# aynik/carta1

Hardware: AMD Instinct MI355X
Metric: atrac1_stereo_frames_per_s_encode (higher is better)
Workload: dtype f32+f64

## Files before the change

### carta1_amd/csrc/c1_api.hip

```cpp
#include <algorithm>
#include <cmath>
#include <cstdarg>
#include <cstdio>
#include <cstdlib>
#include <cstring>
#include <limits>
#include <map>
#include <memory>
#include <atomic>
#include <mutex>
#include <string>
#include <thread>
#include <vector>

#include "c1_internal.h"
#include "c1_detect_bound.h"

#pragma clang fp contract(off)

namespace {

#include "c1_default_tables.inc"

thread_local std::string g_error;
// ... 617 lines not shown
  const bool all_long_modes = !detect && opts->fixed_block_modes[0] == 0 && opts->fixed_block_modes[1] == 0 &&
                              opts->fixed_block_modes[2] == 0 && !getenv("C1_NO_FAST_LONG");
  const bool all_short_modes = !detect && opts->fixed_block_modes[0] != 0 && opts->fixed_block_modes[1] != 0 &&
                               opts->fixed_block_modes[2] != 0;
  bool speculate = (all_long_modes || all_short_modes) && !taps && units && ctx->spec_tables_ok && ctx->spec_mode != 0;
  bool quantize32 = !taps && units && ctx->spec_tables_ok && ctx->spec_mode != 0;
  static const bool det_spec_env_off = getenv("C1_DETECT_SPEC") && atoi(getenv("C1_DETECT_SPEC")) == 0;
  bool detect_spec = detect && !taps && ctx->spec_tables_ok && ctx->spec_mode != 0 && !det_spec_env_off;
  if (ctx->spec_mode == 1 && frames * channels < kSpecMinUnits) speculate = quantize32 = detect_spec = false;
  const bool overlap = speculate && ctx->overlap && ctx->s_tail != nullptr;
  if (!overlap && (rc = join_tail(ctx))) return rc;
  const bool piped = ctx->pipeline && !taps && frames > chunk && !speculate;
  hipStream_t sA = piped ? ctx->s_ana : ctx->stream, sB = piped ? ctx->s_rest : ctx->stream;
  if (piped) {
    HIP_TRY(hipEventRecord(ctx->ev_in, ctx->stream));
    HIP_TRY(hipStreamWaitEvent(sA, ctx->ev_in, 0));
    HIP_TRY(hipStreamWaitEvent(sB, ctx->ev_in, 0));
  }
  int64_t index = 0;
  for (int64_t f0 = 0, n = 0; f0 < frames; f0 += n, ++index) {
    n = taps ? frames : std::min(chunk, frames - f0);
    int p = piped ? (int)(index & 1) : 0;
    if (overlap) { p = ctx->ws_next; ctx->ws_next ^= 1; }
    C1EncodeLaunch L;
    memset(&L, 0, sizeof L);
    for (int c = 0; c < channels; c++) L.pcm[c] = pcm[c] + f0 * 512;
    L.channels = channels;
    L.frames = n;
    L.halo_frames = (int)std::min<int64_t>(2, f0 + halo_frames);
    L.tables = ctx->d_tables;
    L.opts = ctx->d_opts;
    L.coefs = taps ? coefs_tap : ctx->d_coefs[p];
    L.side = taps ? side_tap : ctx->d_side[p];
    L.alloc = taps ? alloc_tap : ctx->d_alloc[p];
    L.cand = ctx->d_cand[p];
    L.work_count = ctx->d_work[p];
    L.work_list = ctx->d_work[p] + 4;
    L.sel_list = ctx->d_work[p] + 4 + (size_t)ctx->ws_units * 7;
    L.bands = bands ? bands + f0 * channels * 512 : nullptr;
    L.units = units ? units + f0 * channels * C1_UNIT_BYTES : nullptr;
    const bool all_long = all_long_modes;
    if (piped && index >= 2) HIP_TRY(hipStreamWaitEvent(sA, ctx->ev_free[p], 0));
    if (speculate) {
      L.eps = ctx->d_eps[p];
      bind_lists(ctx, p, &L);
      if (ctx->spec_mode == 1) { bind_defer(ctx, p, &L); L.spec_defer = ctx->spec_defer; }
      if (c1k_pick_run(n, channels, 0) <= 64 && !getenv("C1_NO_SF_PREPASS"))
        L.open_masks = reinterpret_cast<unsigned long long *>((reinterpret_cast<uintptr_t>(ctx->d_redo[p] + kListHead + 3 * (size_t)ctx->ws_units + (size_t)ctx->ws_units / 4 + 4) + 7) & ~(uintptr_t)7);
      if (overlap && ctx->tail_used[p]) HIP_TRY(hipStreamWaitEvent(sA, ctx->ev_tail[p], 0));
      HIP_TRY(hipMemsetAsync(ctx->d_redo[p], 0, kListHead * sizeof(uint32_t), sA));
      {
        ScopedTiming t(ctx, K_ANALYSIS, sA);
        c1k_launch_analysis_spec(L, all_short_modes, sA);
        if (L.defer_list) {
          C1EncodeLaunch D = L;
          uint32_t *dense = ctx->d_redo[p] + kListHead + 2 * (size_t)ctx->ws_units;
          c1k_launch_defer_compact(L, dense, ctx->d_redo[p] + 3, sA);
          D.unit_list = dense;
          D.unit_count = ctx->d_redo[p] + 3;
          D.list_runs = 1;
          D.defer_list = nullptr;
          if (all_long_modes) c1k_launch_analysis_long(D, sA); else c1k_launch_analysis(D, false, sA);
        }
      }
      if (L.open_masks) {
        ScopedTiming t(ctx, K_REDO, sA);
        {
          C1EncodeLaunch X = L;
          uint32_t *open_list = ctx->d_redo[p] + kListHead + 2 * (size_t)ctx->ws_units;
          c1k_launch_open_compact(L, open_list, ctx->d_redo[p] + 5, sA);
          X.unit_list = open_list;
          X.unit_count = ctx->d_redo[p] + 5;
          X.list_runs = 0;
          X.list_zero_eps = 1;
          X.defer_list = nullptr;
          X.open_masks = nullptr;
          if (all_long_modes) c1k_launch_analysis_long(X, sA); else c1k_launch_analysis(X, false, sA);
        }
      }
      { ScopedTiming t(ctx, K_ALLOCATE, sA); c1k_launch_allocate(L, sA); }
      if (overlap && ctx->tail_used[p ^ 1]) HIP_TRY(hipStreamWaitEvent(sA, ctx->ev_tail[p ^ 1], 0));
      { ScopedTiming t(ctx, K_PACK, sA); c1k_launch_pack_spec(L, all_long_modes, sA); }
      hipStream_t sT = sA;
      if (overlap) {
        sT = ctx->s_tail;
        HIP_TRY(hipEventRecord(ctx->ev_main[p], sA));
        HIP_TRY(hipStreamWaitEvent(sT, ctx->ev_main[p], 0));
      }
      {
        ScopedTiming t(ctx, K_REDO, sT);
        hipStream_t sA = sT;
        C1EncodeLaunch R = L;
        R.defer_list = nullptr;
        R.unit_list = L.reana_list;
        R.unit_count = L.reana_count;
        if (all_long_modes) c1k_launch_analysis_long(R, sA); else c1k_launch_analysis(R, false, sA);
        if (!L.open_masks) {
          C1EncodeLaunch A = R;
          A.unit_list = L.realloc_list;
          A.unit_count = L.realloc_count;
          c1k_launch_allocate(A, sA);
        }
        R.unit_list = L.redo_list;
        R.unit_count = L.redo_count;
        c1k_launch_pack(R, all_long_modes, sA);
        c1k_launch_spec_totals(ctx->d_spec_totals, (uint64_t)(n * channels), ctx->d_redo[p], 0, sA);
      }
      if (overlap) {
        HIP_TRY(hipEventRecord(ctx->ev_tail[p], sT));
        ctx->tail_used[p] = true;
        ctx->tail_pending = true;
      }
      continue;
    }
    {
      ScopedTiming t(ctx, K_ANALYSIS, sA);
      if (all_long) c1k_launch_analysis_long(L, sA);
      else if (detect) {
        c1k_launch_detect(L, ctx->d_bands[p], ctx->d_feat[p], ctx->d_modes[p], ctx->d_lists[p], detect_spec, nullptr, sA);
        if (detect_spec) c1k_launch_spec_totals(ctx->d_spec_totals, (uint64_t)(n * channels), ctx->d_lists[p] + 2, 2, sA);
        if (L.bands) HIP_TRY(hipMemcpyAsync(L.bands, ctx->d_bands[p] + (size_t)channels * 512, (size_t)n * channels * 512 * sizeof(float),
                                            hipMemcpyDeviceToDevice, sA));
      } else c1k_launch_analysis(L, false, sA);
    }
// ... 2787 lines not shown
```

### carta1_amd/csrc/c1_device.h

```cpp
#pragma once
#include "c1_internal.h"

#include <algorithm>
#include <type_traits>

#pragma clang fp contract(off)

#define C1_WAVE 64

typedef const __attribute__((address_space(4))) C1DevTables *TablesPtr;
#define C1_TABLES(p) ((TablesPtr)(p))
__device__ __forceinline__ int lane_for_this_frame(int lane) {
  asm volatile("" : "+v"(lane));
  return lane;
}
__device__ __forceinline__ void wave_fence() {
  __builtin_amdgcn_fence(__ATOMIC_ACQ_REL, "wavefront");
  __builtin_amdgcn_wave_barrier();
}

__device__ __forceinline__ bool own_block() {
  int one = 1;
  asm volatile("" : "+s"(one));
  return one != 0;
// ... 10 lines not shown
__constant__ const uint8_t kSpecs[52] = {8, 8, 8, 8, 4,  4,  4,  4,  8,  8,  8,  8,  6,  6,  6,  6,  6,  6,
                                   6, 6, 6, 6, 6,  6,  7,  7,  7,  7,  9,  9,  9,  9,  10, 10, 10, 10,
                                   12, 12, 12, 12, 12, 12, 12, 12, 20, 20, 20, 20, 20, 20, 20, 20};
__constant__ const uint16_t kStartLong[52] = {0,   8,   16,  24,  32,  36,  40,  44,  48,  56,  64,  72,  80,
                                        86,  92,  98,  104, 110, 116, 122, 128, 134, 140, 146, 152, 159,
                                        166, 173, 180, 189, 198, 207, 216, 226, 236, 246, 256, 268, 280,
                                        292, 304, 316, 328, 340, 352, 372, 392, 412, 432, 452, 472, 492};
__constant__ const uint16_t kStartShort[52] = {0,   32,  64,  96,  8,   40,  72,  104, 12,  44,  76,  108, 20,
                                         52,  84,  116, 26,  58,  90,  122, 128, 160, 192, 224, 134, 166,
                                         198, 230, 141, 173, 205, 237, 150, 182, 214, 246, 256, 288, 320,
                                         352, 384, 416, 448, 480, 268, 300, 332, 364, 396, 428, 460, 492};
__constant__ const uint16_t kBfuFirst[53] = {0,   8,   16,  24,  32,  36,  40,  44,  48,  56,  64,  72,  80,  86,
                                       92,  98,  104, 110, 116, 122, 128, 134, 140, 146, 152, 159, 166, 173,
                                       180, 189, 198, 207, 216, 226, 236, 246, 256, 268, 280, 292, 304, 316,
                                       328, 340, 352, 372, 392, 412, 432, 452, 472, 492, 512};
__device__ __forceinline__ int bfu_amount(int index) { return index == 0 ? 20 : 24 + 4 * index; }

__device__ __forceinline__ int wl_bits(int wl) { return wl == 0 ? 0 : wl + 1; }
__device__ __forceinline__ int band_of_bfu(int b) { return b >= 36 ? 2 : (b >= 20 ? 1 : 0); }
__device__ __forceinline__ int bfu_of_slot(int p) {
  if (p < 32) return p >> 3;
  if (p < 48) return 4 + ((p - 32) >> 2);
  if (p < 80) return 8 + ((p - 48) >> 3);
  if (p < 152) return 12 + (p - 80) / 6;
  if (p < 180) return 24 + (p - 152) / 7;
  if (p < 216) return 28 + (p - 180) / 9;
  if (p < 256) return 32 + (p - 216) / 10;
  if (p < 352) return 36 + (p - 256) / 12;
  return 44 + (p - 352) / 20;
}

__device__ __forceinline__ float f32(double x) { return (float)x; }
typedef float v4f __attribute__((ext_vector_type(4)));

__device__ __forceinline__ int32_t to_int32(double x) {
  const double t = trunc(x);
  if (fabs(t) < 2147483648.0) return (int32_t)t;
  const uint64_t bits = (uint64_t)__double_as_longlong(t);
  const int e = (int)((bits >> 52) & 0x7ff);
  if (e == 0x7ff) return 0;
  const int sh = e - 1075;
  const uint64_t mant = (bits & 0xfffffffffffffull) | (1ull << 52);
  uint32_t low;
  if (sh >= 32) low = 0u;
  else if (sh >= 0) low = (uint32_t)(mant << sh);
  else low = (uint32_t)(mant >> (-sh));
  return (int32_t)((bits >> 63) ? (0u - low) : low);
}


template <int S = 5>
__device__ __forceinline__ int pidx(int e) { return e + ((e >> S) << 1); }

template <int D, int S>
__device__ __forceinline__ const double2 *qmf_window(const double *w, int lane, int u) {
  if constexpr (2 * D == (1 << S)) return reinterpret_cast<const double2 *>(w + (2 * D + 2) * lane + (2 * u + 2 * ((2 * u) >> S)));
  else return reinterpret_cast<const double2 *>(&w[pidx<S>(2 * D * lane + 2 * u)]);
}
template <int D, int S = 5>
__device__ __forceinline__ void qmf_analysis_core(const double *w, int lane, TablesPtr T,
                                                  double (&even)[D], double (&odd)[D]) {
#pragma unroll
  for (int d = 0; d < D; d++) even[d] = odd[d] = 0.0;
#pragma unroll
  for (int u = 22 + D; u >= 0; --u) {
    const double2 x = *qmf_window<D, S>(w, lane, u);
#pragma unroll
    for (int d = 0; d < D; d++) {
      const int j = d + 23 - u;
      if (j >= 0 && j < 24) {
        odd[d] = __builtin_fma(x.x, T->tap_e[23 - j], odd[d]);
        even[d] = __builtin_fma(x.y, T->tap_e[j], even[d]);
      }
    }
  }
}
template <int D, int S = 5>
__device__ __forceinline__ void qmf_synthesis_core(const double *w, int lane, TablesPtr T,
                                                   double (&s0)[D], double (&s1)[D]) {
#pragma unroll
  for (int d = 0; d < D; d++) s0[d] = s1[d] = 0.0;
#pragma unroll
  for (int u = 0; u <= 22 + D; ++u) {
    const double2 x = *qmf_window<D, S>(w, lane, u);
#pragma unroll
    for (int d = 0; d < D; d++) {
      const int j = u - d;
      if (j >= 0 && j < 24) {
        s0[d] = __builtin_fma(x.x, T->tap_e[j], s0[d]);
        s1[d] = __builtin_fma(x.y, T->tap_e[23 - j], s1[d]);
      }
    }
  }
}

__device__ __forceinline__ int wave_inclusive_scan(int x) {
  x += __builtin_amdgcn_update_dpp(0, x, 0x111, 0xf, 0xf, false);
  x += __builtin_amdgcn_update_dpp(0, x, 0x112, 0xf, 0xf, false);
  x += __builtin_amdgcn_update_dpp(0, x, 0x114, 0xf, 0xf, false);
  x += __builtin_amdgcn_update_dpp(0, x, 0x118, 0xf, 0xf, false);
  x += __builtin_amdgcn_update_dpp(0, x, 0x142, 0xa, 0xf, false);
  x += __builtin_amdgcn_update_dpp(0, x, 0x143, 0xc, 0xf, false);
  return x;
}

__device__ __forceinline__ int bitrev(int k, int log2n) { return (int)(__brev((unsigned)k) >> (32 - log2n)); }

__device__ __forceinline__ int scale_factor_index_fast(float maxabs, uint32_t m1, uint32_t m2) {
  const uint32_t u = __float_as_uint(maxabs);
// ... 491 lines not shown
```

### carta1_amd/csrc/c1_internal.h

```cpp
#pragma once

#include <hip/hip_runtime.h>
#include <stdint.h>
#include <stdlib.h>

#include "../../include/carta1_hip.h"

struct C1DevTables {
  double tap_e[24];
  double tap_o[24];
  double window[32];
  double mdct_fwd64[32];
  double mdct_fwd256[128];
  double mdct_fwd512[256];
  double mdct_inv64[32];
  double mdct_inv256[128];
  double mdct_inv512[256];
  double fft_tw[256][2];
  double scale_factors[64];
  double norm[64 * 16];
  double log1p10;
  uint32_t sf_m1, sf_m2;
  int32_t sf_fast;
  int32_t dq_fast;
// ... 149 lines not shown
  if (hipOccupancyMaxActiveBlocksPerMultiprocessor(&per_cu, kernel, 64, 0) != hipSuccess || per_cu <= 0) per_cu = 8;
  if (hipGetDevice(&dev) != hipSuccess || hipDeviceGetAttribute(&cus, hipDeviceAttributeMultiprocessorCount, dev) != hipSuccess || cus <= 0) cus = 256;
  return per_cu * cus;
}

void c1k_launch_analysis(const C1EncodeLaunch &L, bool detect, hipStream_t stream);
void c1k_launch_analysis_long(const C1EncodeLaunch &L, hipStream_t stream);
void c1k_launch_analysis_spec(const C1EncodeLaunch &L, bool all_short, hipStream_t stream);
constexpr int kFeatureWsDoubles = 20;
void c1k_launch_detect(const C1EncodeLaunch &L, float *bands_ws, double *feat_ws, uint8_t *modes_ws, uint32_t *lists_ws,
                       bool speculative, double *score_tap, hipStream_t stream);
void c1k_launch_mdct_bands(const C1EncodeLaunch &L, const float *bands_ws, const uint8_t *modes_ws, const uint32_t *lists_ws, hipStream_t stream);
void c1k_launch_unpack_units(const uint8_t *units, int64_t frames, int32_t *nbfu, int32_t *modes, int32_t *sfi, int32_t *wl,
                             int32_t *q, hipStream_t stream);
void c1k_launch_dequantize_frames(const C1DevTables *tables, const int32_t *nbfu, const int32_t *modes, const int32_t *sfi,
                                  const int32_t *wl, const int32_t *q, int64_t frames, float *coefs, hipStream_t stream);
void c1k_launch_imdct_frames(const C1DevTables *tables, const float *coefs, const int32_t *modes, int64_t frames, int halo,
                             float *bands, hipStream_t stream);
void c1k_launch_qmf_synthesis_frames(const C1DevTables *tables, const float *bands, int64_t frames, int halo, float *pcm,
                                     hipStream_t stream);
void c1k_launch_block_modes_from_bands(const C1DevTables *tables, const float *bands, int64_t frames, int halo, double threshold,
                                       float *mags, int32_t *modes, hipStream_t stream);
void c1k_launch_stage_mode_lists(const int32_t *modes, int64_t frames, uint8_t *mode_bytes, uint32_t *lists, hipStream_t stream);
void c1k_launch_stage_scale_factors(const C1DevTables *tables, const float *coefs, const int32_t *modes, int64_t frames, uint8_t *side,
                                    hipStream_t stream);
void c1k_launch_stage_fields(const C1DevTables *tables, const float *coefs, const int32_t *modes, const uint8_t *side,
                             const uint8_t *alloc, int64_t frames, int32_t *nbfu, int32_t *sfi, int32_t *wl, int32_t *q,
                             hipStream_t stream);
void c1k_launch_pack_units(const int32_t *nbfu, const int32_t *modes, const int32_t *sfi, const int32_t *wl, const int32_t *q,
                           int64_t frames, uint8_t *units, hipStream_t stream);
void c1k_launch_quantize_one(const C1DevTables *tables, const float *x, int n, int sfi, int bits, int32_t *out, hipStream_t stream);
void c1k_launch_dequantize_one(const C1DevTables *tables, const int32_t *q, int n, int sfi, int bits, float *out, hipStream_t stream);
void c1k_launch_fft_reference(float *real, float *imag, int n, const double *w, double *twiddle_scratch , hipStream_t stream);
void c1k_launch_window_bands(const float *bands, const uint8_t *modes, int64_t units, const C1DevTables *tables, float *out, hipStream_t stream);
void c1k_launch_js_log2(const double *in, double *out, int64_t n, hipStream_t stream);
void c1k_launch_find_scale_factors(const double *values, const int64_t *offsets, const int64_t *counts, int64_t problems, int32_t *out,
                                   hipStream_t stream);
void c1k_launch_perform_fft(const double *samples, const int64_t *offsets, int64_t problems, int n, const double *w, double *tw,
                            float *re, float *im, float *mag, hipStream_t stream);
void c1k_launch_detect_transients(const double *cur, const int64_t *cur_off, const double *prev, const int64_t *prev_off,
                                  const uint8_t *has_prev, const double *thresholds, int64_t problems, const C1DevTables *tables,
                                  uint8_t *transient, double *scores, hipStream_t stream);
void c1k_launch_allocate_bits(const double *data, const int64_t *bfu_off, const int32_t *bfu_len, const int32_t *bfu_sizes,
                              const int32_t *max_bfus, int64_t problems, const double *bsf, int32_t *count, int32_t *wl, int32_t *sfi,
                              uint8_t *fallback, hipStream_t stream);
void c1k_launch_detect_spec_tap(const C1EncodeLaunch &L, float *bands_ws, double *feat_ws, hipStream_t stream);
void c1k_launch_libm(int fn, const double *in, double *out, int64_t n, hipStream_t stream);
void c1k_launch_log2f_error(uint32_t first, uint64_t count, unsigned long long *out, hipStream_t stream);
void c1k_launch_allocate(const C1EncodeLaunch &L, hipStream_t stream);
void c1k_launch_alloc_tap(const C1EncodeLaunch &L, double *out, hipStream_t stream);
void c1k_launch_pack(const C1EncodeLaunch &L, bool all_long, hipStream_t stream);
void c1k_launch_pack_spec(const C1EncodeLaunch &L, bool all_long, hipStream_t stream);
void c1k_launch_spec_totals(unsigned long long *totals, uint64_t units, const uint32_t *counts, int kind, hipStream_t stream);
void c1k_launch_defer_compact(const C1EncodeLaunch &L, uint32_t *list, uint32_t *counts, hipStream_t stream);
void c1k_launch_open_compact(const C1EncodeLaunch &L, uint32_t *list, uint32_t *count, hipStream_t stream);
void c1k_launch_decode(const C1DecodeLaunch &L, bool binary32, hipStream_t stream);
void c1k_launch_decode_fields(const C1DecodeFieldsLaunch &L, hipStream_t stream);
void c1k_launch_encode_from_states(const C1EncStateLaunch &L, hipStream_t stream);
void c1k_launch_decode_from_states(const C1DecStateLaunch &L, hipStream_t stream);
void c1k_launch_encode_rows(const C1EncStateLaunch &L, hipStream_t stream);
void c1k_launch_decode_rows(const C1DecStateLaunch &L, hipStream_t stream);
void c1k_launch_copy_rows(uint32_t *dst, const uint32_t *dst_rows, const uint32_t *src, const uint32_t *src_rows, int src_broadcast,
                          int64_t n, int dwords, hipStream_t stream);
void c1k_launch_state_mags(const C1DevTables *tables, const float *bands, int64_t rows, float *states, hipStream_t stream);
void c1k_launch_generate_white(const uint32_t *frame_states, int64_t frames, float *pcm, int kind_mask, double amp, hipStream_t stream);
void c1k_launch_generate_pink(const uint32_t *segment_states, int64_t frames, float *pcm, int kind_mask, hipStream_t stream);
void c1k_launch_generate_sines(int64_t frames, float *pcm, int kind_mask, uint32_t seed, hipStream_t stream);
void c1k_launch_pcm_from_int(const void *src, int bits, int channels, int64_t n, float *const *pcm, hipStream_t stream);
void c1k_launch_pcm_to_int16(const float *const *pcm, int channels, int64_t n, int16_t *dst, hipStream_t stream);
```

### carta1_amd/csrc/c1_k_analysis.hip

```cpp
#include "c1_device.h"

namespace {

struct alignas(16) LongLds {
  float d1[46];
  float d2[46];
  uint32_t late[4][64];
  uint32_t sfw[64];
  double win[32];
  alignas(16) float hbuf[296];
  alignas(4) uint8_t sfi[64];
  union alignas(16) {
    struct { alignas(16) double w1[698]; } q1;
    struct { alignas(16) double w2[454]; } q2;
    struct {
      union alignas(16) {
        struct { alignas(16) float in0[256]; alignas(16) float in1[256]; alignas(16) float in2[512]; } i;
        struct { alignas(16) float coef[512]; } c;
      } a;
      union alignas(16) { float band[512]; } zz;
    } m;
    struct { alignas(16) float skip_[896]; float2 z[320]; } zp;
  } u;
};
// ... 25 lines not shown
  float *band_;
  if constexpr (ALL_LONG) band_ = S.u.m.zz.band; else band_ = S.band;
  const C1DevEncOpts *O = L.opts;
  const int lane0 = threadIdx.x;
  int lane = lane0;
  const bool listed = L.unit_list != nullptr;
  const int64_t n_items = listed ? (int64_t)*L.unit_count : (int64_t)gridDim.x;
  R4Geometry G4 = r4_geometry(lane0);
  const SfLong SFL = sf_long_geometry(lane0);
  if constexpr (ALL_LONG) {
#pragma unroll
    for (int j = 0; j < 4; j++) {
      S.late[j][lane0] = r4_late_word(G4, j);
      G4.cx[j] = G4.cy[j] = G4.post_tab[j] = 0;
    }
    S.sfw[lane0] = (uint32_t)SFL.src | ((uint32_t)SFL.b << 13) | (SFL.wide ? 1u << 19 : 0u) | (SFL.store ? 1u << 20 : 0u);
    if (lane0 < 32) S.win[lane0] = C1_TABLES(L.tables)->window[lane0];
  }
  const SfLong SFM = sf_geometry(lane0, O->modes[0], O->modes[1], O->modes[2]);
  const MixGeometry GM = mix_geometry(lane0, FrameModes{O->modes[0], O->modes[1], O->modes[2]});
  const TablesRsrc RT = tables_rsrc(L.tables);
  for (int64_t item = blockIdx.x; item < n_items; item += gridDim.x) {
  const int64_t listed_unit = listed ? (int64_t)L.unit_list[item] : 0;
  const int ch = listed ? (int)(listed_unit % L.channels) : (int)(blockIdx.x % L.channels);
  const int64_t f0 = listed ? listed_unit / L.channels : (int64_t)(blockIdx.x / L.channels) * L.run_frames;
  const int64_t run_frames = listed ? (L.list_runs ? (f0 / L.run_frames + 1) * L.run_frames - f0 : 1) : L.run_frames;
  const float *__restrict__ pcm = L.pcm[ch];
  lane = lane0;

  for (int i = lane; i < 46; i += 64) { S.d1[i] = 0.0; S.d2[i] = 0.0; }
  for (int i = lane; i < 296; i += 64) S.hbuf[i] = 0.0f;
  if (lane < 12) S.sfi[52 + lane] = 0;
  if constexpr (!ALL_LONG) {
    for (int i = lane; i < 96; i += 64) S.ovl[i] = 0.0f;
  }
  float ov0 = 0.0f, ov1 = 0.0f, ov2 = 0.0f;
  wave_fence();

  const int64_t f_end = (f0 + run_frames < L.frames) ? f0 + run_frames : L.frames;
  constexpr int kWarm = 1;
  int64_t f_first = f0 - kWarm;
  if (f_first < -(int64_t)L.halo_frames) f_first = -(int64_t)L.halo_frames;
  if (f_first > f0) f_first = f0;
  typedef float v4f __attribute__((ext_vector_type(4)));
  v4f pre_a, pre_b;
  auto deliver = [&]() {
    asm volatile("" : "+v"(pre_a), "+v"(pre_b));
  };
  {
    const v4f *p4 = reinterpret_cast<const v4f *>(pcm + f_first * 512);
    pre_a = p4[lane0]; pre_b = p4[64 + lane0];
    deliver();
  }
  for (int64_t f = f_first; f < f_end; ++f) {
    const bool emit = (f >= f0);
    TablesPtr T = tables_for_this_frame(L.tables);
    lane = lane_for_this_frame(lane0);

    {
      const v4f a = pre_a, b = pre_b;
      {
        const v4f *p4 = reinterpret_cast<const v4f *>(pcm + ((f + 1 < f_end) ? f + 1 : f) * 512);
        pre_a = p4[lane]; pre_b = p4[64 + lane];
      }
      double *w1 = S.u.q1.w1;
      if (lane < 46) w1[pidx<3>(lane)] = S.d1[lane];
      const int e0 = 46 + 4 * lane;
      *reinterpret_cast<double2 *>(&w1[pidx<3>(e0)]) = make_double2((double)a.x, (double)a.y);
      *reinterpret_cast<double2 *>(&w1[pidx<3>(e0 + 2)]) = make_double2((double)a.z, (double)a.w);
      *reinterpret_cast<double2 *>(&w1[pidx<3>(e0 + 256)]) = make_double2((double)b.x, (double)b.y);
      *reinterpret_cast<double2 *>(&w1[pidx<3>(e0 + 258)]) = make_double2((double)b.z, (double)b.w);
    }
    wave_fence();
    {
      double ev[4], od[4];
      if constexpr (ALL_LONG) __builtin_amdgcn_s_setprio(3);
      if (own_block()) qmf_analysis_core<4, 3>(S.u.q1.w1, lane, T, ev, od); else { for (int d = 0; d < 4; d++) { ev[d] = S.u.q1.w1[lane + d]; od[d] = 1.0; } }
      double *w2 = S.u.q2.w2;
      if (lane < 46) { w2[pidx<2>(lane)] = S.d2[lane]; S.d1[lane] = S.u.q1.w1[pidx<3>(512 + lane)]; }
      float lo[4];
#pragma unroll
      for (int d = 0; d < 4; d++) {
        lo[d] = f32(ev[d] + od[d]);
        S.hbuf[39 + 4 * lane + d] = f32(ev[d] - od[d]);
      }
      *reinterpret_cast<double2 *>(&w2[pidx<2>(46 + 4 * lane)]) = make_double2((double)lo[0], (double)lo[1]);
      *reinterpret_cast<double2 *>(&w2[pidx<2>(48 + 4 * lane)]) = make_double2((double)lo[2], (double)lo[3]);
    }
    wave_fence();
    R4Early EARLY;
    if constexpr (ALL_LONG) EARLY = r4_early(G4, RT);
    {
      double ev[2], od[2];
      if (own_block()) qmf_analysis_core<2, 2>(S.u.q2.w2, lane, T, ev, od); else { for (int d = 0; d < 2; d++) { ev[d] = S.u.q2.w2[lane + d]; od[d] = 1.0; } }
      if constexpr (ALL_LONG) __builtin_amdgcn_s_setprio(1);
      *reinterpret_cast<float2 *>(&band_[2 * lane]) = make_float2(f32(ev[0] + od[0]), f32(ev[1] + od[1]));
      *reinterpret_cast<float2 *>(&band_[128 + 2 * lane]) = make_float2(f32(ev[0] - od[0]), f32(ev[1] - od[1]));
      *reinterpret_cast<float4 *>(&band_[256 + 4 * lane]) = *reinterpret_cast<const float4 *>(&S.hbuf[4 * lane]);
      if (lane < 46) S.d2[lane] = S.u.q2.w2[pidx<2>(256 + lane)];
    }
    wave_fence();
    {
      float keep = 0.0f;
      if (lane < 39) keep = S.hbuf[256 + lane];
      wave_fence();
      if (lane < 39) S.hbuf[lane] = keep;
    }
    deliver();
    if (emit && L.bands) {
      float4 *dst = reinterpret_cast<float4 *>(L.bands + ((f * L.channels + ch) << 9));
      const float4 *src = reinterpret_cast<const float4 *>(band_);
      dst[lane] = src[lane];
      dst[64 + lane] = src[64 + lane];
    }

    if constexpr (ALL_LONG) {
      float *in0 = S.u.m.a.i.in0, *in1 = S.u.m.a.i.in1, *in2 = S.u.m.a.i.in2;
      float nov0 = 0.0f, nov1 = 0.0f, nov2 = 0.0f;
      if (lane < 32) {
        const double w_lo = S.win[lane], w_hi = S.win[31 - lane];
        const double x0 = band_[96 + lane], x1 = band_[128 + 96 + lane], x2 = band_[256 + 224 + lane];
        nov0 = f32(w_lo * x0); nov1 = f32(w_lo * x1); nov2 = f32(w_lo * x2);
        if (emit) {
          in0[48 + lane] = ov0; in1[48 + lane] = ov1; in2[112 + lane] = ov2;
          in0[80 + 96 + lane] = f32(x0 * w_hi);
          in1[80 + 96 + lane] = f32(x1 * w_hi);
          in2[144 + 224 + lane] = f32(x2 * w_hi);
        }
      }
      ov0 = nov0; ov1 = nov1; ov2 = nov2;
      if (!emit) { wave_fence(); continue; }
      {
        const float4 zero4 = make_float4(0.0f, 0.0f, 0.0f, 0.0f);
        if (lane < 48) {
          float *inb = lane < 24 ? in0 : in1;
          const int q = lane < 24 ? lane : lane - 24;
          *reinterpret_cast<float4 *>(&inb[q < 12 ? 4 * q : 208 + 4 * (q - 12)]) = zero4;
        }
        if (lane < 56) *reinterpret_cast<float4 *>(&in2[lane < 28 ? 4 * lane : 400 + 4 * (lane - 28)]) = zero4;
        if (lane < 48) {
          *reinterpret_cast<float2 *>(&in0[80 + 2 * lane]) = *reinterpret_cast<const float2 *>(&band_[2 * lane]);
          *reinterpret_cast<float2 *>(&in1[80 + 2 * lane]) = *reinterpret_cast<const float2 *>(&band_[128 + 2 * lane]);
        }
        if (lane < 56) *reinterpret_cast<float4 *>(&in2[144 + 4 * lane]) = *reinterpret_cast<const float4 *>(&band_[256 + 4 * lane]);
      }
      wave_fence();
      float *coef = S.u.m.a.c.coef;
      __builtin_amdgcn_s_setprio(0);
      mdct_long_r4(in0, S.u.zp.z, coef, G4, T, RT, EARLY, &S.late[0][0] + lane);
      __builtin_amdgcn_s_setprio(1);
      wave_fence();

      const int64_t unit = f * L.channels + ch;
      {
        const uint32_t sw = S.sfw[lane];
        const float4 *grp = reinterpret_cast<const float4 *>(coef + (sw & 0x1fcu));
        float mx = sf_scan_long_groups(grp[0], grp[1], grp[2]);
        const float other = __int_as_float(__builtin_amdgcn_update_dpp(0, __float_as_int(mx), 0xB1, 0xf, 0xf, false));
        mx = fmaxf(mx, ((sw >> 19) & 1u) ? other : 0.0f);
        const int sfi = scale_factor_index_fast(mx, T->sf_m1, T->sf_m2);
        if ((sw >> 20) & 1u) S.sfi[(sw >> 13) & 63u] = (uint8_t)sfi;
      }
      {
        float4 *dst = reinterpret_cast<float4 *>(L.coefs + (unit << 9));
        const float4 *src = reinterpret_cast<const float4 *>(coef);
        dst[lane] = src[lane];
        dst[64 + lane] = src[64 + lane];
      }
      wave_fence();
      if (lane < 16) reinterpret_cast<uint32_t *>(L.side + unit * kSideBytes)[lane] = reinterpret_cast<const uint32_t *>(S.sfi)[lane];
      if ((L.list_runs || L.list_zero_eps) && lane == 16) *reinterpret_cast<float4 *>(L.eps + unit * kEpsFloats) = make_float4(0.0f, 0.0f, 0.0f, 0.0f);
      wave_fence();
    } else {
      const FrameModes M{O->modes[0], O->modes[1], O->modes[2]};
      float *coef = S.u.m.a.c.coef;
      if (emit) {
        mix_stage(band_, S.ovl, S.u.m.a.g.in, M, lane, RT);
        wave_fence();
        mdct_mixed_r4(S.u.m.a.g.in, S.u.m.zz.z, coef, GM, M.m0 == 0 || M.m1 == 0 || M.m2 == 0, M.m2 == 0, T, RT);
      }
      for (int i = lane; i < 96; i += 64) {
        const int b = i >> 5, k = i & 31;
        const int Sb = b == 2 ? 256 : 128, off = b == 0 ? 0 : (b == 1 ? 128 : 256);
        S.ovl[i] = f32(T->window[k] * (double)band_[off + Sb - 32 + k]);
      }
      wave_fence();
      if (!emit) continue;

      const int64_t unit = f * L.channels + ch;
      {
        float4 *dst = reinterpret_cast<float4 *>(L.coefs + (unit << 9));
        const float4 *src = reinterpret_cast<const float4 *>(coef);
        dst[lane] = src[lane];
        dst[64 + lane] = src[64 + lane];
      }
      sf_long(coef, S.sfi, SFM, T);
      if (lane >= 60 && lane < 63) reinterpret_cast<uint32_t *>(S.sfi)[13 + (lane - 60)] = lane == 60 ? (uint32_t)((M.m0 & 3) | ((M.m1 & 3) << 2) | ((M.m2 & 3) << 4)) : 0u;
      wave_fence();
      if (lane < 16) reinterpret_cast<uint32_t *>(L.side + unit * kSideBytes)[lane] = reinterpret_cast<const uint32_t *>(S.sfi)[lane];
      if ((L.list_runs || L.list_zero_eps) && lane == 16) *reinterpret_cast<float4 *>(L.eps + unit * kEpsFloats) = make_float4(0.0f, 0.0f, 0.0f, 0.0f);
      wave_fence();
    }
  }
  wave_fence();
  }
}

}

void c1k_launch_analysis(const C1EncodeLaunch &L0, bool detect, hipStream_t stream) {
  static const int slots = c1k_wave_slots(k_analysis_fast<false>);
  C1EncodeLaunch L = L0;
  L.run_frames = c1k_pick_run(L.frames, L.channels, slots);
  const int64_t runs = (L.frames + L.run_frames - 1) / L.run_frames;
  const int64_t blocks = L.unit_list ? std::min<int64_t>(L.frames * L.channels, 256 * 12) : runs * L.channels;
  const dim3 grid((unsigned)blocks), block(C1_WAVE);
  (void)detect;
  hipLaunchKernelGGL((k_analysis_fast<false>), grid, block, 0, stream, L);
}
void c1k_launch_analysis_long(const C1EncodeLaunch &L0, hipStream_t stream) {
  static const int slots = c1k_wave_slots(k_analysis_fast<true>);
  C1EncodeLaunch L = L0;
  L.run_frames = c1k_pick_run(L.frames, L.channels, slots);
  const int64_t runs = (L.frames + L.run_frames - 1) / L.run_frames;
  const int64_t blocks = L.unit_list ? std::min<int64_t>(L.frames * L.channels, 256 * 16) : runs * L.channels;
  hipLaunchKernelGGL((k_analysis_fast<true>), dim3((unsigned)blocks), dim3(C1_WAVE), 0, stream, L);
}
static_assert(sizeof(LongLds) <= 10240, "all-long analysis: 16 waves per CU (4 per SIMD, 128 registers) need <= 10 KiB of LDS per wave");
```

### carta1_amd/csrc/c1_k_spec.hip

```cpp
#include "c1_device.h"

namespace {

constexpr int kR2 = 840;
constexpr int kMemFloats = kR2 + 576;
constexpr int kIn2 = 1;
struct alignas(16) SpecLds {
  alignas(16) float mem[kMemFloats];
  alignas(16) float d1[48];
  alignas(16) float d2[48];
  alignas(16) float pre2[76];
  alignas(4) uint8_t sfi[64];
  uint32_t geo[3][64];
};
constexpr int kSpecWaves = 4;
constexpr int kSpecTabBase = (int)offsetof(C1DevTables, win32);
constexpr int kSpecTabFloats = ((int)offsetof(C1DevTables, r2d) + (int)sizeof(((C1DevTables *)nullptr)->r2d) - kSpecTabBase) / 4;
static_assert(offsetof(C1DevTables, pre32_64) > offsetof(C1DevTables, win32) && offsetof(C1DevTables, r2d) > offsetof(C1DevTables, r4c) &&
              offsetof(C1DevTables, norm32) == offsetof(C1DevTables, r2d) + sizeof(((C1DevTables *)nullptr)->r2d), "win32 .. r2d are one contiguous block");
static_assert(kSpecWaves * sizeof(SpecLds) + kSpecTabFloats * 4 + 27 * 16 <= 32768, "speculative analysis: 5 workgroups of 4 waves per CU");
constexpr int kE2 = 0, kH2 = 288, kE0 = kR2, kH0 = kR2 + 160, kE1 = kR2 + 288, kH1 = kR2 + 448;

__device__ __forceinline__ int w1_phys(int v) { return __mul24(12, v >> 3) + (v & 7); }

// ... 485 lines not shown
      const v4f *src = reinterpret_cast<const v4f *>(coef);
      const int lq = lane_for_this_frame(lane0);
      __builtin_nontemporal_store(src[lq], &dst[lq]);
      __builtin_nontemporal_store(src[64 + lq], &dst[64 + lq]);
    }
    const float Z0 = __builtin_amdgcn_sqrtf(lane_value(zrow, 0)), Z1 = __builtin_amdgcn_sqrtf(lane_value(zrow, 16));
    const float Z2 = __builtin_amdgcn_sqrtf(SHORT ? fmaxf(lane_value(zrow, 32), lane_value(zrow, 48)) : lane_value(zrow, 32) + lane_value(zrow, 48));
    const float eabs = T->spec_eabs;
    const float cz0 = SHORT ? T->spec_cz_short[0] : T->spec_cz[0], cz1 = SHORT ? T->spec_cz_short[1] : T->spec_cz[1], cz2 = SHORT ? T->spec_cz_short[2] : T->spec_cz[2];
    const float cw0 = SHORT ? T->spec_cw_short[0] : T->spec_cw[0], cw1 = SHORT ? T->spec_cw_short[1] : T->spec_cw[1], cw2 = SHORT ? T->spec_cw_short[2] : T->spec_cw[2];
    const float cl0 = SHORT ? T->spec_cl_short[0] : T->spec_cl[0], cl1 = SHORT ? T->spec_cl_short[1] : T->spec_cl[1], cl2 = SHORT ? T->spec_cl_short[2] : T->spec_cl[2];
    const float e0 = __builtin_fmaf(cz0, Z0, __builtin_fmaf(cw0, W, __builtin_fmaf(cl0, Lw, eabs)));
    const float e1 = __builtin_fmaf(cz1, Z1, __builtin_fmaf(cw1, W, __builtin_fmaf(cl1, Lw, eabs)));
    const float e2 = __builtin_fmaf(cz2, Z2, __builtin_fmaf(cw2, W, __builtin_fmaf(cl2, Lw, eabs)));
    bool unstable;
    {
      SfLong SFL = SFL0;
      float mx = 0.0f;
      if constexpr (SHORT) {
        asm volatile("" : "+v"(SFL.src), "+v"(SFL.cnt));
        const float *src = coef + SFL.src;
#pragma unroll
        for (int j = 0; j < 12; j++) mx = fmaxf(mx, fabsf(src[j < SFL.cnt ? j : SFL.cnt - 1]));
      } else {
        const uint32_t sw = S.geo[0][lane];
        SFL.b = (int)((sw >> 9) & 63u);
        SFL.wide = ((sw >> 15) & 1u) != 0u;
        SFL.store = ((sw >> 16) & 1u) != 0u;
        const float4 *grp = reinterpret_cast<const float4 *>(coef + (sw & 0x1ffu));
        mx = sf_scan_long_groups(grp[0], grp[1], grp[2]);
      }
      const float other = __int_as_float(__builtin_amdgcn_update_dpp(0, __float_as_int(mx), 0xB1, 0xf, 0xf, false));
      mx = fmaxf(mx, SFL.wide ? other : 0.0f);
      const float e = SFL.b >= 36 ? e2 : (SFL.b >= 20 ? e1 : e0);
      const float lo = fmaxf((mx - e) * 0.99999976f, 0.0f), hi = (mx + e) * 1.00000024f;
      const int s_lo = scale_factor_index_fast(lo, T->sf_m1, T->sf_m2), s_hi = scale_factor_index_fast(hi, T->sf_m1, T->sf_m2);
      if (SFL.store) S.sfi[SFL.b] = (uint8_t)s_lo;
      unstable = lane < 60 && !(s_lo == s_hi && e < __builtin_huge_valf());
    }
    const bool any_unstable = __builtin_amdgcn_ballot_w64(unstable) != 0;
    wave_fence();
    if (L.defer_list != nullptr && (((int)(f - f0)) & (kSpecCheckFrames - 1)) == 0) {
      if (spec_should_defer(S.sfi, lane, e0, e1, e2, L.opts, L.spec_defer)) { deferred_from = (uint32_t)unit; break; }
    }
    if (any_unstable) open_bits |= 1ull << (int)((f - f0) & 63);
    if (lane < 16) reinterpret_cast<uint32_t *>(L.side + unit * kSideBytes)[lane] = reinterpret_cast<const uint32_t *>(S.sfi)[lane];
    if (lane == 0) *reinterpret_cast<float4 *>(L.eps + unit * kEpsFloats) = make_float4(e0, e1, e2, __int_as_float(any_unstable ? 1 : 0));
    wave_fence();
  }
  if (L.defer_list != nullptr && lane0 == 0) L.defer_list[slot] = deferred_from;
  if (L.open_masks != nullptr && lane0 == 0) L.open_masks[slot] = open_bits;
}

__global__ __launch_bounds__(256) void k_defer_compact(const uint32_t *__restrict__ slots, uint32_t n_slots, uint32_t *__restrict__ list, uint32_t *__restrict__ counts,
                                                        int channels, int run_frames, uint32_t frames) {
  const uint32_t i = blockIdx.x * 256u + threadIdx.x;
  const uint32_t u = i < n_slots ? slots[i] : 0xffffffffu;
  const bool on = u != 0xffffffffu;
  uint32_t covered = 0;
  if (on) {
    const uint32_t f = u / (uint32_t)channels;
    uint32_t end = (f / (uint32_t)run_frames + 1u) * (uint32_t)run_frames;
    if (end > frames) end = frames;
    covered = end - f;
  }
  const uint64_t mask = __builtin_amdgcn_ballot_w64(on);
  if (mask == 0) return;
  int cov = (int)covered;
  cov = wave_inclusive_scan(cov);
  const int lane = threadIdx.x & 63;
  uint32_t at = 0;
  if (lane == 63) {
    at = atomicAdd(counts, (uint32_t)__popcll(mask));
    atomicAdd(counts + 1, (uint32_t)cov);
  }
  at = (uint32_t)__builtin_amdgcn_readlane((int)at, 63);
  if (on) list[at + __popcll(mask & ((1ull << lane) - 1ull))] = u;
}

__global__ __launch_bounds__(256) void k_open_compact(const unsigned long long *__restrict__ masks, uint32_t n_slots, uint32_t *__restrict__ list,
                                                       uint32_t *__restrict__ count, int channels, int run_frames) {
  const uint32_t i = blockIdx.x * 256u + threadIdx.x;
  unsigned long long m = i < n_slots ? masks[i] : 0ull;
  const int mine = __popcll(m);
  if (__builtin_amdgcn_ballot_w64(mine != 0) == 0) return;
  const int scan = wave_inclusive_scan(mine);
  const int lane = threadIdx.x & 63;
  uint32_t at = 0;
  if (lane == 63) at = atomicAdd(count, (uint32_t)scan);
  at = (uint32_t)__builtin_amdgcn_readlane((int)at, 63) + (uint32_t)(scan - mine);
  const uint32_t run = i / (uint32_t)channels, ch = i % (uint32_t)channels;
  while (m != 0ull) {
    const int k = __ffsll((long long)m) - 1;
    m &= m - 1ull;
    list[at++] = (run * (uint32_t)run_frames + (uint32_t)k) * (uint32_t)channels + ch;
  }
}

__global__ void k_spec_totals(unsigned long long *totals, unsigned long long units, const uint32_t *counts, int kind) {
  if (kind == 0) {
    const unsigned long long deferred = counts[4];
    totals[0] += units - deferred;
    totals[1] += counts[2] + counts[5];
    totals[2] += deferred;
    totals[3] += counts[0] - counts[2];
    totals[6] += deferred;
  } else if (kind == 1) {
    totals[2] += units;
    totals[3] += counts[0];
  } else {
    totals[4] += units;
    totals[5] += counts[0];
  }
}

}

void c1k_launch_spec_totals(unsigned long long *totals, uint64_t units, const uint32_t *counts, int kind, hipStream_t stream) {
  hipLaunchKernelGGL(k_spec_totals, dim3(1), dim3(1), 0, stream, totals, (unsigned long long)units, counts, kind);
}
void c1k_launch_open_compact(const C1EncodeLaunch &L, uint32_t *list, uint32_t *count, hipStream_t stream) {
  const int run = c1k_pick_run(L.frames, L.channels, 0);
  const int64_t slots = (L.frames + run - 1) / run * L.channels;
  hipLaunchKernelGGL(k_open_compact, dim3((unsigned)((slots + 255) / 256)), dim3(256), 0, stream, (const unsigned long long *)L.open_masks, (uint32_t)slots, list, count,
                     L.channels, run);
}
void c1k_launch_defer_compact(const C1EncodeLaunch &L, uint32_t *list, uint32_t *counts, hipStream_t stream) {
  const int run = c1k_pick_run(L.frames, L.channels, 0);
  const int64_t slots = (L.frames + run - 1) / run * L.channels;
  hipLaunchKernelGGL(k_defer_compact, dim3((unsigned)((slots + 255) / 256)), dim3(256), 0, stream, (const uint32_t *)L.defer_list, (uint32_t)slots, list, counts,
                     L.channels, run, (uint32_t)L.frames);
}

void c1k_launch_analysis_spec(const C1EncodeLaunch &L0, bool all_short, hipStream_t stream) {
  static const int slots = c1k_wave_slots(k_analysis_spec<false>);
  C1EncodeLaunch L = L0;
  L.run_frames = c1k_pick_run(L.frames, L.channels, slots);
  const int64_t runs = (L.frames + L.run_frames - 1) / L.run_frames, n_slots = runs * L.channels;
  const dim3 grid((unsigned)((n_slots + kSpecWaves - 1) / kSpecWaves)), block(C1_WAVE * kSpecWaves);
  static const bool no_spread = getenv("C1_NO_SPREAD") != nullptr;
  L.spread_bits = 0;
  if (!no_spread) while ((1ll << L.spread_bits) < (int64_t)grid.x) L.spread_bits++;
  if (all_short) hipLaunchKernelGGL((k_analysis_spec<true>), grid, block, 0, stream, L);
  else hipLaunchKernelGGL((k_analysis_spec<false>), grid, block, 0, stream, L);
}
```

Baseline: 186.9 million.

## Fuse defer/open list compaction into one kernel and peel warm-up analysis frame

Replaces the separate defer-compact and open-compact kernels with a single launch that builds both lists. The lists now go into L.realloc_list and L.reana_list instead of sharing one scratch region, so the compaction can happen once, before the deferred analysis pass. Separately, the warm-up (non-emitting) frame in the analysis kernel is peeled out of the main loop into a reduced QMF-only prologue, which removes the per-frame emit branches. This trims launch overhead and loop divergence, but relies on realloc_list and reana_list being bound and not aliasing other buffers.

```diff
diff --git a/carta1_amd/csrc/c1_api.hip b/carta1_amd/csrc/c1_api.hip
--- a/carta1_amd/csrc/c1_api.hip
+++ b/carta1_amd/csrc/c1_api.hip
@@ -693,11 +693,10 @@
       {
         ScopedTiming t(ctx, K_ANALYSIS, sA);
         c1k_launch_analysis_spec(L, all_short_modes, sA);
+        if (L.defer_list || L.open_masks) c1k_launch_lists_compact(L, L.realloc_list, ctx->d_redo[p] + 3, L.reana_list, ctx->d_redo[p] + 5, sA);
         if (L.defer_list) {
           C1EncodeLaunch D = L;
-          uint32_t *dense = ctx->d_redo[p] + kListHead + 2 * (size_t)ctx->ws_units;
-          c1k_launch_defer_compact(L, dense, ctx->d_redo[p] + 3, sA);
-          D.unit_list = dense;
+          D.unit_list = L.realloc_list;
           D.unit_count = ctx->d_redo[p] + 3;
           D.list_runs = 1;
           D.defer_list = nullptr;
@@ -708,9 +707,7 @@
         ScopedTiming t(ctx, K_REDO, sA);
         {
           C1EncodeLaunch X = L;
-          uint32_t *open_list = ctx->d_redo[p] + kListHead + 2 * (size_t)ctx->ws_units;
-          c1k_launch_open_compact(L, open_list, ctx->d_redo[p] + 5, sA);
-          X.unit_list = open_list;
+          X.unit_list = L.reana_list;
           X.unit_count = ctx->d_redo[p] + 5;
           X.list_runs = 0;
           X.list_zero_eps = 1;
diff --git a/carta1_amd/csrc/c1_device.h b/carta1_amd/csrc/c1_device.h
--- a/carta1_amd/csrc/c1_device.h
+++ b/carta1_amd/csrc/c1_device.h
@@ -86,9 +86,11 @@
 template <int S = 5>
 __device__ __forceinline__ int pidx(int e) { return e + ((e >> S) << 1); }
 
+constexpr int kQmfFlat = 0;
 template <int D, int S>
 __device__ __forceinline__ const double2 *qmf_window(const double *w, int lane, int u) {
-  if constexpr (2 * D == (1 << S)) return reinterpret_cast<const double2 *>(w + (2 * D + 2) * lane + (2 * u + 2 * ((2 * u) >> S)));
+  if constexpr (S == kQmfFlat) return reinterpret_cast<const double2 *>(w + 2 * D * lane + 2 * u);
+  else if constexpr (2 * D == (1 << S)) return reinterpret_cast<const double2 *>(w + (2 * D + 2) * lane + (2 * u + 2 * ((2 * u) >> S)));
   else return reinterpret_cast<const double2 *>(&w[pidx<S>(2 * D * lane + 2 * u)]);
 }
 template <int D, int S = 5>
diff --git a/carta1_amd/csrc/c1_internal.h b/carta1_amd/csrc/c1_internal.h
--- a/carta1_amd/csrc/c1_internal.h
+++ b/carta1_amd/csrc/c1_internal.h
@@ -225,8 +225,7 @@
 void c1k_launch_pack(const C1EncodeLaunch &L, bool all_long, hipStream_t stream);
 void c1k_launch_pack_spec(const C1EncodeLaunch &L, bool all_long, hipStream_t stream);
 void c1k_launch_spec_totals(unsigned long long *totals, uint64_t units, const uint32_t *counts, int kind, hipStream_t stream);
-void c1k_launch_defer_compact(const C1EncodeLaunch &L, uint32_t *list, uint32_t *counts, hipStream_t stream);
-void c1k_launch_open_compact(const C1EncodeLaunch &L, uint32_t *list, uint32_t *count, hipStream_t stream);
+void c1k_launch_lists_compact(const C1EncodeLaunch &L, uint32_t *run_list, uint32_t *run_counts, uint32_t *open_list, uint32_t *open_count, hipStream_t stream);
 void c1k_launch_decode(const C1DecodeLaunch &L, bool binary32, hipStream_t stream);
 void c1k_launch_decode_fields(const C1DecodeFieldsLaunch &L, hipStream_t stream);
 void c1k_launch_encode_from_states(const C1EncStateLaunch &L, hipStream_t stream);
diff --git a/carta1_amd/csrc/c1_k_analysis.hip b/carta1_amd/csrc/c1_k_analysis.hip
--- a/carta1_amd/csrc/c1_k_analysis.hip
+++ b/carta1_amd/csrc/c1_k_analysis.hip
@@ -101,8 +101,59 @@
     pre_a = p4[lane0]; pre_b = p4[64 + lane0];
     deliver();
   }
-  for (int64_t f = f_first; f < f_end; ++f) {
-    const bool emit = (f >= f0);
+  if (f_first < f0) {
+    TablesPtr T = tables_for_this_frame(L.tables);
+    lane = lane_for_this_frame(lane0);
+    double *w1 = S.u.q1.w1;
+    double *w2 = S.u.q1.w1 + 456;
+    {
+      const v4f a = pre_a, b = pre_b;
+      {
+        const v4f *p4 = reinterpret_cast<const v4f *>(pcm + f0 * 512);
+        pre_a = p4[lane]; pre_b = p4[64 + lane];
+      }
+      const int ea = 4 * lane - 210, eb = 46 + 4 * lane;
+      if (lane > 52) *reinterpret_cast<double2 *>(&w1[pidx<2>(ea)]) = make_double2((double)a.x, (double)a.y);
+      if (lane >= 52) *reinterpret_cast<double2 *>(&w1[pidx<2>(ea + 2)]) = make_double2((double)a.z, (double)a.w);
+      *reinterpret_cast<double2 *>(&w1[pidx<2>(eb)]) = make_double2((double)b.x, (double)b.y);
+      *reinterpret_cast<double2 *>(&w1[pidx<2>(eb + 2)]) = make_double2((double)b.z, (double)b.w);
+    }
+    wave_fence();
+    {
+      double ev[2], od[2];
+      if constexpr (ALL_LONG) __builtin_amdgcn_s_setprio(3);
+      if (own_block()) qmf_analysis_core<2, 2>(w1, lane, T, ev, od); else { for (int d = 0; d < 2; d++) { ev[d] = w1[lane + d]; od[d] = 1.0; } }
+      if (lane < 46) S.d1[lane] = w1[pidx<2>(256 + lane)];
+      const float lo0 = f32(ev[0] + od[0]), lo1 = f32(ev[1] + od[1]);
+      S.hbuf[39 + 128 + 2 * lane] = f32(ev[0] - od[0]);
+      S.hbuf[39 + 129 + 2 * lane] = f32(ev[1] - od[1]);
+      if (lane >= 9) *reinterpret_cast<double2 *>(&w2[2 * lane - 18]) = make_double2((double)lo0, (double)lo1);
+    }
+    wave_fence();
+    {
+      double ev[1] = {0.0}, od[1] = {0.0};
+      if (lane < 32) qmf_analysis_core<1, kQmfFlat>(w2, lane, T, ev, od);
+      if constexpr (ALL_LONG) __builtin_amdgcn_s_setprio(1);
+      if (lane < 46) S.d2[lane] = w2[64 + lane];
+      if (lane < 32) {
+        const double x0 = f32(ev[0] + od[0]), x1 = f32(ev[0] - od[0]), x2 = S.hbuf[224 + lane];
+        if constexpr (ALL_LONG) {
+          const double w_lo = S.win[lane];
+          ov0 = f32(w_lo * x0); ov1 = f32(w_lo * x1); ov2 = f32(w_lo * x2);
+        } else {
+          const double w_lo = T->window[lane];
+          S.ovl[lane] = f32(w_lo * x0); S.ovl[32 + lane] = f32(w_lo * x1); S.ovl[64 + lane] = f32(w_lo * x2);
+        }
+      }
+      float keep = 0.0f;
+      if (lane < 39) keep = S.hbuf[256 + lane];
+      wave_fence();
+      if (lane < 39) S.hbuf[lane] = keep;
+    }
+    wave_fence();
+    deliver();
+  }
+  for (int64_t f = f0; f < f_end; ++f) {
     TablesPtr T = tables_for_this_frame(L.tables);
     lane = lane_for_this_frame(lane0);
 
@@ -156,7 +207,7 @@
       if (lane < 39) S.hbuf[lane] = keep;
     }
     deliver();
-    if (emit && L.bands) {
+    if (L.bands) {
       float4 *dst = reinterpret_cast<float4 *>(L.bands + ((f * L.channels + ch) << 9));
       const float4 *src = reinterpret_cast<const float4 *>(band_);
       dst[lane] = src[lane];
@@ -170,15 +221,12 @@
         const double w_lo = S.win[lane], w_hi = S.win[31 - lane];
         const double x0 = band_[96 + lane], x1 = band_[128 + 96 + lane], x2 = band_[256 + 224 + lane];
         nov0 = f32(w_lo * x0); nov1 = f32(w_lo * x1); nov2 = f32(w_lo * x2);
-        if (emit) {
-          in0[48 + lane] = ov0; in1[48 + lane] = ov1; in2[112 + lane] = ov2;
-          in0[80 + 96 + lane] = f32(x0 * w_hi);
-          in1[80 + 96 + lane] = f32(x1 * w_hi);
-          in2[144 + 224 + lane] = f32(x2 * w_hi);
-        }
+        in0[48 + lane] = ov0; in1[48 + lane] = ov1; in2[112 + lane] = ov2;
+        in0[80 + 96 + lane] = f32(x0 * w_hi);
+        in1[80 + 96 + lane] = f32(x1 * w_hi);
+        in2[144 + 224 + lane] = f32(x2 * w_hi);
       }
       ov0 = nov0; ov1 = nov1; ov2 = nov2;
-      if (!emit) { wave_fence(); continue; }
       {
         const float4 zero4 = make_float4(0.0f, 0.0f, 0.0f, 0.0f);
         if (lane < 48) {
@@ -223,18 +271,15 @@
     } else {
       const FrameModes M{O->modes[0], O->modes[1], O->modes[2]};
       float *coef = S.u.m.a.c.coef;
-      if (emit) {
-        mix_stage(band_, S.ovl, S.u.m.a.g.in, M, lane, RT);
-        wave_fence();
-        mdct_mixed_r4(S.u.m.a.g.in, S.u.m.zz.z, coef, GM, M.m0 == 0 || M.m1 == 0 || M.m2 == 0, M.m2 == 0, T, RT);
-      }
+      mix_stage(band_, S.ovl, S.u.m.a.g.in, M, lane, RT);
+      wave_fence();
+      mdct_mixed_r4(S.u.m.a.g.in, S.u.m.zz.z, coef, GM, M.m0 == 0 || M.m1 == 0 || M.m2 == 0, M.m2 == 0, T, RT);
       for (int i = lane; i < 96; i += 64) {
         const int b = i >> 5, k = i & 31;
         const int Sb = b == 2 ? 256 : 128, off = b == 0 ? 0 : (b == 1 ? 128 : 256);
         S.ovl[i] = f32(T->window[k] * (double)band_[off + Sb - 32 + k]);
       }
       wave_fence();
-      if (!emit) continue;
 
       const int64_t unit = f * L.channels + ch;
       {
diff --git a/carta1_amd/csrc/c1_k_spec.hip b/carta1_amd/csrc/c1_k_spec.hip
--- a/carta1_amd/csrc/c1_k_spec.hip
+++ b/carta1_amd/csrc/c1_k_spec.hip
@@ -561,48 +561,49 @@
   if (L.open_masks != nullptr && lane0 == 0) L.open_masks[slot] = open_bits;
 }
 
-__global__ __launch_bounds__(256) void k_defer_compact(const uint32_t *__restrict__ slots, uint32_t n_slots, uint32_t *__restrict__ list, uint32_t *__restrict__ counts,
+__global__ __launch_bounds__(256) void k_lists_compact(const uint32_t *__restrict__ slots, const unsigned long long *__restrict__ masks, uint32_t n_slots,
+                                                        uint32_t *__restrict__ run_list, uint32_t *__restrict__ run_counts,
+                                                        uint32_t *__restrict__ open_list, uint32_t *__restrict__ open_count,
                                                         int channels, int run_frames, uint32_t frames) {
   const uint32_t i = blockIdx.x * 256u + threadIdx.x;
-  const uint32_t u = i < n_slots ? slots[i] : 0xffffffffu;
-  const bool on = u != 0xffffffffu;
-  uint32_t covered = 0;
-  if (on) {
-    const uint32_t f = u / (uint32_t)channels;
-    uint32_t end = (f / (uint32_t)run_frames + 1u) * (uint32_t)run_frames;
-    if (end > frames) end = frames;
-    covered = end - f;
-  }
-  const uint64_t mask = __builtin_amdgcn_ballot_w64(on);
-  if (mask == 0) return;
-  int cov = (int)covered;
-  cov = wave_inclusive_scan(cov);
   const int lane = threadIdx.x & 63;
-  uint32_t at = 0;
-  if (lane == 63) {
-    at = atomicAdd(counts, (uint32_t)__popcll(mask));
-    atomicAdd(counts + 1, (uint32_t)cov);
-  }
-  at = (uint32_t)__builtin_amdgcn_readlane((int)at, 63);
-  if (on) list[at + __popcll(mask & ((1ull << lane) - 1ull))] = u;
-}
-
-__global__ __launch_bounds__(256) void k_open_compact(const unsigned long long *__restrict__ masks, uint32_t n_slots, uint32_t *__restrict__ list,
-                                                       uint32_t *__restrict__ count, int channels, int run_frames) {
-  const uint32_t i = blockIdx.x * 256u + threadIdx.x;
-  unsigned long long m = i < n_slots ? masks[i] : 0ull;
-  const int mine = __popcll(m);
-  if (__builtin_amdgcn_ballot_w64(mine != 0) == 0) return;
-  const int scan = wave_inclusive_scan(mine);
-  const int lane = threadIdx.x & 63;
-  uint32_t at = 0;
-  if (lane == 63) at = atomicAdd(count, (uint32_t)scan);
-  at = (uint32_t)__builtin_amdgcn_readlane((int)at, 63) + (uint32_t)(scan - mine);
-  const uint32_t run = i / (uint32_t)channels, ch = i % (uint32_t)channels;
-  while (m != 0ull) {
-    const int k = __ffsll((long long)m) - 1;
-    m &= m - 1ull;
-    list[at++] = (run * (uint32_t)run_frames + (uint32_t)k) * (uint32_t)channels + ch;
+  if (slots != nullptr) {
+    const uint32_t u = i < n_slots ? slots[i] : 0xffffffffu;
+    const bool on = u != 0xffffffffu;
+    uint32_t covered = 0;
+    if (on) {
+      const uint32_t f = u / (uint32_t)channels;
+      uint32_t end = (f / (uint32_t)run_frames + 1u) * (uint32_t)run_frames;
+      if (end > frames) end = frames;
+      covered = end - f;
+    }
+    const uint64_t mask = __builtin_amdgcn_ballot_w64(on);
+    if (mask != 0) {
+      int cov = (int)covered;
+      cov = wave_inclusive_scan(cov);
+      uint32_t at = 0;
+      if (lane == 63) {
+        at = atomicAdd(run_counts, (uint32_t)__popcll(mask));
+        atomicAdd(run_counts + 1, (uint32_t)cov);
+      }
+      at = (uint32_t)__builtin_amdgcn_readlane((int)at, 63);
+      if (on) run_list[at + __popcll(mask & ((1ull << lane) - 1ull))] = u;
+    }
+  }
+  if (masks != nullptr) {
+    unsigned long long m = i < n_slots ? masks[i] : 0ull;
+    const int mine = __popcll(m);
+    if (__builtin_amdgcn_ballot_w64(mine != 0) == 0) return;
+    const int scan = wave_inclusive_scan(mine);
+    uint32_t at = 0;
+    if (lane == 63) at = atomicAdd(open_count, (uint32_t)scan);
+    at = (uint32_t)__builtin_amdgcn_readlane((int)at, 63) + (uint32_t)(scan - mine);
+    const uint32_t run = i / (uint32_t)channels, ch = i % (uint32_t)channels;
+    while (m != 0ull) {
+      const int k = __ffsll((long long)m) - 1;
+      m &= m - 1ull;
+      open_list[at++] = (run * (uint32_t)run_frames + (uint32_t)k) * (uint32_t)channels + ch;
+    }
   }
 }
 
@@ -628,17 +629,11 @@
 void c1k_launch_spec_totals(unsigned long long *totals, uint64_t units, const uint32_t *counts, int kind, hipStream_t stream) {
   hipLaunchKernelGGL(k_spec_totals, dim3(1), dim3(1), 0, stream, totals, (unsigned long long)units, counts, kind);
 }
-void c1k_launch_open_compact(const C1EncodeLaunch &L, uint32_t *list, uint32_t *count, hipStream_t stream) {
+void c1k_launch_lists_compact(const C1EncodeLaunch &L, uint32_t *run_list, uint32_t *run_counts, uint32_t *open_list, uint32_t *open_count, hipStream_t stream) {
   const int run = c1k_pick_run(L.frames, L.channels, 0);
   const int64_t slots = (L.frames + run - 1) / run * L.channels;
-  hipLaunchKernelGGL(k_open_compact, dim3((unsigned)((slots + 255) / 256)), dim3(256), 0, stream, (const unsigned long long *)L.open_masks, (uint32_t)slots, list, count,
-                     L.channels, run);
-}
-void c1k_launch_defer_compact(const C1EncodeLaunch &L, uint32_t *list, uint32_t *counts, hipStream_t stream) {
-  const int run = c1k_pick_run(L.frames, L.channels, 0);
-  const int64_t slots = (L.frames + run - 1) / run * L.channels;
-  hipLaunchKernelGGL(k_defer_compact, dim3((unsigned)((slots + 255) / 256)), dim3(256), 0, stream, (const uint32_t *)L.defer_list, (uint32_t)slots, list, counts,
-                     L.channels, run, (uint32_t)L.frames);
+  hipLaunchKernelGGL(k_lists_compact, dim3((unsigned)((slots + 255) / 256)), dim3(256), 0, stream, (const uint32_t *)L.defer_list,
+                     (const unsigned long long *)L.open_masks, (uint32_t)slots, run_list, run_counts, open_list, open_count, L.channels, run, (uint32_t)L.frames);
 }
 
 void c1k_launch_analysis_spec(const C1EncodeLaunch &L0, bool all_short, hipStream_t stream) {
```

Result: no change. 187.4 million (median of 2 runs) (+0.3%).
